# Voyager0587/yolov8-vit

Measured on AMD Instinct MI355X. Metric: images/sec end-to-end (640->224 detect+classify), higher is better.
Workload: dtype bf16; 1 GPU; YOLOv8n(nc=5)+ViT-B/16 end-to-end inference, 640x640, bf16 (BASELINE.json configs[1]); batch_per_gpu=32, global_batch=32, crops_per_image=4, parallelism=dp1, weights=random-init, seed 42

## Files before the change

include/yv_hip.h:

```cpp
#ifndef YV_HIP_H
#define YV_HIP_H

#include <stddef.h>
#include <stdint.h>

#ifdef __cplusplus
extern "C" {
#endif

#define YV_OK 0
#define YV_ERR_ARG (-1)
#define YV_ERR_LIMIT (-2)
#define YV_ERR_WORKSPACE (-3)
#define YV_ERR_LAUNCH (-4)

int yv_version(void);
const char* yv_error_string(int code);
int yv_device_is_gfx950(void);
int yv_set_option(const char* key, int value);
int yv_get_option(const char* key, int* value);

int yv_linear_mxfp8_q(const void* Aq, long long lda, const void* Ascale, long long a_rows_pad, const void* Wq, const void* Wscale,
                      long long w_rows_pad, const float* bias, int M, int N, int K, int flags, const int32_t* m_dev, int m_mul,
                      void* out_q, long long ldq, void* out_scales, long long out_rows_pad, void* stream);
// ... 168 lines not shown
} yv_mx_view;

int yv_quant_mxfp8_map(const void* x, long long ldx, long long pixels, int C, void* q, long long ldq, void* scales,
                       void* stream);

int yv_conv2d_mxfp8(const yv_mx_view* in0, const yv_mx_view* in1, int B, int Hout, int Wout, int ksize, int stride,
                    const void* wq, const void* wscale, long long w_rows_pad, const float* bias, int Cout, void* out_bf16,
                    int out_ld, void* out_q, void* out_scales, int outq_ld, const void* res, int res_ld, int flags,
                    void* stream);
int yv_conv2d_mxfp8_instance(int B, int Hout, int Wout, int ksize, int stride, int Cin, int Cout);

int yv_c2f_fused(const void* x, long long ldx, int B, int H, int W, int c, int n, const void* w_cv1, const float* b_cv1,
                 const void* const* w_m, const float* const* b_m, const void* w_cv2, const float* b_cv2, void* out,
                 long long ldo, void* stream);
int yv_c2f_debug(void* buf);

int yv_conv2d_ws(const yv_view* in0, const yv_view* in1, int B, int Hout, int Wout, int ksize, int stride,
                 const void* weight, const float* bias, int Cout, void* out, int out_ld, const void* res, int res_ld,
                 int flags, void* ws, size_t ws_bytes, void* stream);

int yv_conv2d_stats(const yv_view* in0, int B, int Hout, int Wout, int ksize, int stride, const void* weight,
                    const float* bias, int Cout, void* out, int out_ld, int flags, float* stats_ws, size_t stats_ws_floats,
                    void* ws, size_t ws_bytes, void* stream);
size_t yv_conv_stats_ws_floats(long long T, int Cout);

int yv_conv2d_bnbwd(const yv_view* in0, int B, int Hout, int Wout, int ksize, int stride, const void* weight, const float* bias,
                    int Cout, void* out, int out_ld, const void* res, int res_ld, int flags, const void* z, int ldz,
                    const float* mean, const float* rstd, const float* gamma, const float* beta, int act, float* stats_ws,
                    size_t stats_ws_floats, void* ws, size_t ws_bytes, void* stream);
size_t yv_conv_bnbwd_ws_floats(long long T, int Cout);
// ... 194 lines not shown
```

yolov8-vit_amd/csrc/c2f.hip:

```cpp
#include "yv_common.h"

namespace {

struct C2fArgs {
    const uint16_t* x; long long ldx;
    int B, H, W, tiles_x, tiles_y;
    const uint16_t* w_cv1; const float* b_cv1;
    const uint16_t* w_m[4]; const float* b_m[4];
    const uint16_t* w_cv2; const float* b_cv2;
    uint16_t* out; long long ldo;
    unsigned long long* dbg;
};

__device__ __forceinline__ float c2f_silu(float x) { return x * __builtin_amdgcn_rcpf(1.0f + __expf(-x)); }

typedef __attribute__((ext_vector_type(4))) uint32_t c2f_u32x4;

__device__ __forceinline__ bf16x8 c2f_zero8() { return __builtin_bit_cast(bf16x8, (c2f_u32x4){0u, 0u, 0u, 0u}); }

template <int C, int NB, int TT> struct C2fGeo {
    static constexpr int C2F_T = TT;
    static constexpr int HALO = 2 * NB, R0 = C2F_T + 2 * HALO, PXB = C * 2;
    static constexpr int y_w(int j) { return j == 0 ? C2F_T : R0 - 4 * (j - 1); }
    static constexpr int t_w(int j) { return R0 - 2 - 4 * j; }
    static constexpr int y_off(int j) {
        int o = 0;
        for (int i = 0; i < j; ++i) o += y_w(i) * y_w(i) * PXB + (i >= 1 && i <= NB ? t_w(i - 1) * t_w(i - 1) * PXB : 0);
        return o;
    }
    static constexpr int t_off(int j) { return y_off(j + 1) + y_w(j + 1) * y_w(j + 1) * PXB; }
    static constexpr int BYTES = y_off(NB + 1) + y_w(NB + 1) * y_w(NB + 1) * PXB;
};

template <int C> struct C2fConvW {
    static constexpr int CPG = C / 8, KG = 9 * CPG, KS = (KG + 3) / 4, NFR = C / 16;
    bf16x8 wa[NFR][KS];
    float4 bv[NFR];
};
template <int C>
__device__ __forceinline__ void c2f_load_conv_w(C2fConvW<C>& w, const uint16_t* __restrict__ wgt, const float* __restrict__ bias, int r,
                                                int q) {
    using CW = C2fConvW<C>;
#pragma unroll
    for (int ks = 0; ks < CW::KS; ++ks) {
        const int kg = 4 * ks + q;
#pragma unroll
        for (int f = 0; f < CW::NFR; ++f)
            w.wa[f][ks] = kg < CW::KG ? *(const bf16x8*)(wgt + (size_t)(16 * f + r) * (9 * C) + 8 * kg) : c2f_zero8();
    }
#pragma unroll
    for (int f = 0; f < CW::NFR; ++f) w.bv[f] = *(const float4*)(bias + 16 * f + 4 * q);
}

template <int C, int NTH, bool RES>
__device__ __forceinline__ void c2f_conv3(const C2fConvW<C>& w, const unsigned char* S, int ws, unsigned char* D,
                                          const unsigned char* Rs, int oy, int ox, int H, int W, int lane, int wave) {
    using CW = C2fConvW<C>;
    constexpr int CPG = CW::CPG, KG = CW::KG, KS = CW::KS, NFR = CW::NFR, NW = NTH / 64;
    const int r = lane & 15, q = lane >> 4;
    const int wd = ws - 2, npd = wd * wd, nps = ws * ws, wr = ws + 2;
    int off[KS];
    uint32_t vmask = 0;
#pragma unroll
    for (int ks = 0; ks < KS; ++ks) {
        const int kg = 4 * ks + q;
        const bool valid = kg < KG;
        const int tap = kg / CPG, plane = kg - tap * CPG;
        off[ks] = valid ? ((tap / 3) * ws + (tap % 3) + plane * nps) * 16 : 0;
        vmask |= valid ? 1u << ks : 0u;
    }
    const int ngroups = (npd + 15) >> 4;
    for (int g0 = wave; g0 < ngroups; g0 += 2 * NW) {
        int p_[2], py_[2], px_[2];
        bool live_[2];
        bf16x8 xb[2][KS];
#pragma unroll
        for (int u = 0; u < 2; ++u) {
            const int g = g0 + u * NW;
            live_[u] = g < ngroups;
            const int p = (live_[u] ? g : g0) * 16 + r;
            const int pc = p < npd ? p : npd - 1;
            p_[u] = p; py_[u] = pc / wd; px_[u] = pc - py_[u] * wd;
            const int sbase = (py_[u] * ws + px_[u]) * 16;
#pragma unroll
            for (int ks = 0; ks < KS; ++ks) {
                xb[u][ks] = *(const bf16x8*)(S + sbase + off[ks]);
                if constexpr ((KG & 3) != 0) { if (ks == KS - 1 && !((vmask >> ks) & 1)) xb[u][ks] = c2f_zero8(); }
            }
        }
        f32x4 acc[2][NFR];
#pragma unroll
        for (int u = 0; u < 2; ++u)
#pragma unroll
            for (int f = 0; f < NFR; ++f) acc[u][f] = (f32x4){0.f, 0.f, 0.f, 0.f};
#pragma unroll
        for (int ks = 0; ks < KS; ++ks)
#pragma unroll
            for (int u = 0; u < 2; ++u)
#pragma unroll
                for (int f = 0; f < NFR; ++f)
                    acc[u][f] = __builtin_amdgcn_mfma_f32_16x16x32_bf16(w.wa[f][ks], xb[u][ks], acc[u][f], 0, 0, 0);
#pragma unroll
        for (int u = 0; u < 2; ++u) {
            const int p = p_[u], py = py_[u], px = px_[u];
            const int iy = oy + py, ix = ox + px;
            const bool inimg = iy >= 0 && iy < H && ix >= 0 && ix < W;
#pragma unroll
            for (int f = 0; f < NFR; ++f) {
                const int ch0 = 16 * f + 4 * q;
                float v[4] = {c2f_silu(acc[u][f][0] + w.bv[f].x), c2f_silu(acc[u][f][1] + w.bv[f].y), c2f_silu(acc[u][f][2] + w.bv[f].z),
                              c2f_silu(acc[u][f][3] + w.bv[f].w)};
                if constexpr (RES) {
                    const uint2 rr = *(const uint2*)(Rs + ((ch0 >> 3) * (wr * wr) + (py + 2) * wr + (px + 2)) * 16 + ((ch0 >> 2) & 1) * 8);
                    v[0] += bf16_to_f32((uint16_t)(rr.x & 0xffff)); v[1] += bf16_to_f32((uint16_t)(rr.x >> 16));
                    v[2] += bf16_to_f32((uint16_t)(rr.y & 0xffff)); v[3] += bf16_to_f32((uint16_t)(rr.y >> 16));
                }
                uint2 pk = make_uint2(pack_bf16x2(v[0], v[1]), pack_bf16x2(v[2], v[3]));
                if (!inimg) pk = make_uint2(0u, 0u);
                if (live_[u] && p < npd) *(uint2*)(D + ((ch0 >> 3) * npd + p) * 16 + ((ch0 >> 2) & 1) * 8) = pk;
            }
        }
    }
}

constexpr int C2F_NTH = 256;

template <int C, int NB, int TT>
__global__ __launch_bounds__(C2F_NTH) void c2f_fused_kernel(C2fArgs a) {
    using G = C2fGeo<C, NB, TT>;
    constexpr int T = TT, HALO = G::HALO, R0 = G::R0, CPG = C / 8, C1 = 2 * C, NTH = C2F_NTH, NW = NTH / 64;
    extern __shared__ __attribute__((aligned(16))) unsigned char smem[];
    const int tid = threadIdx.x, lane = tid & 63, wave = __builtin_amdgcn_readfirstlane(tid >> 6);
    const int r = lane & 15, q = lane >> 4;
    int bid = blockIdx.x;
    const int tx = bid % a.tiles_x; bid /= a.tiles_x;
    const int ty = bid % a.tiles_y;
    const int b = bid / a.tiles_y;
    const int H = a.H, W = a.W;
    const int oy = ty * T - HALO, ox = tx * T - HALO;

    C2fConvW<C> wA, wB;
    unsigned long long st_[8] = {0, 0, 0, 0, 0, 0, 0, 0};
    int sti = 0;
    auto stamp = [&]() __attribute__((always_inline)) { if (a.dbg) st_[sti] = __builtin_readcyclecounter(); ++sti; };
    stamp();
    {
        constexpr int NFR = C1 / 16, KS = C1 / 32, N0 = R0 * R0, NG = (N0 + 15) / 16, MAXG = (NG + NW - 1) / NW;
        bf16x8 xb[MAXG][KS];
#pragma unroll
        for (int i = 0; i < MAXG; ++i) {
            const int p = (wave + i * NW) * 16 + r;
            const int py = p / R0, px = p - py * R0;
            const int iy = oy + py, ix = ox + px;
            const bool inimg = p < N0 && iy >= 0 && iy < H && ix >= 0 && ix < W;
            const uint16_t* src = a.x + (((long long)b * H + (inimg ? iy : 0)) * W + (inimg ? ix : 0)) * a.ldx + 8 * q;
#pragma unroll
            for (int ks = 0; ks < KS; ++ks) xb[i][ks] = inimg ? *(const bf16x8*)(src + 32 * ks) : c2f_zero8();
        }
        bf16x8 wa[NFR][KS];
        float4 bv[NFR];
#pragma unroll
        for (int f = 0; f < NFR; ++f) {
#pragma unroll
            for (int ks = 0; ks < KS; ++ks) wa[f][ks] = *(const bf16x8*)(a.w_cv1 + (size_t)(16 * f + r) * C1 + 32 * ks + 8 * q);
            bv[f] = *(const float4*)(a.b_cv1 + 16 * f + 4 * q);
        }
        c2f_load_conv_w<C>(wA, a.w_m[0], a.b_m[0], r, q);
        unsigned char* Y0 = smem + G::y_off(0);
        unsigned char* Y1 = smem + G::y_off(1);
#pragma unroll
        for (int i = 0; i < MAXG; ++i) {
            const int p = (wave + i * NW) * 16 + r;
            const int py = p / R0, px = p - py * R0;
            const int iy = oy + py, ix = ox + px;
            const bool inimg = p < N0 && iy >= 0 && iy < H && ix >= 0 && ix < W;
            f32x4 acc[NFR];
#pragma unroll
            for (int f = 0; f < NFR; ++f) acc[f] = (f32x4){0.f, 0.f, 0.f, 0.f};
#pragma unroll
            for (int ks = 0; ks < KS; ++ks)
#pragma unroll
                for (int f = 0; f < NFR; ++f) acc[f] = __builtin_amdgcn_mfma_f32_16x16x32_bf16(wa[f][ks], xb[i][ks], acc[f], 0, 0, 0);
            const bool centre = py >= HALO && py < HALO + T && px >= HALO && px < HALO + T;
#pragma unroll
            for (int f = 0; f < NFR; ++f) {
                const int ch0 = 16 * f + 4 * q;
                uint2 pk = make_uint2(pack_bf16x2(c2f_silu(acc[f][0] + bv[f].x), c2f_silu(acc[f][1] + bv[f].y)),
                                      pack_bf16x2(c2f_silu(acc[f][2] + bv[f].z), c2f_silu(acc[f][3] + bv[f].w)));
                if (!inimg) pk = make_uint2(0u, 0u);
                if (ch0 < C) {
                    if (centre && p < N0) *(uint2*)(Y0 + ((ch0 >> 3) * (T * T) + (py - HALO) * T + (px - HALO)) * 16 + ((ch0 >> 2) & 1) * 8) = pk;
                } else if (p < N0) {
                    const int c0 = ch0 - C;
                    *(uint2*)(Y1 + ((c0 >> 3) * N0 + p) * 16 + ((c0 >> 2) & 1) * 8) = pk;
                }
            }
        }
    }
    constexpr int NFR2 = C1 / 16, KG2 = (2 + NB) * CPG, KS2 = (KG2 + 3) / 4, KC2 = (2 + NB) * C;
    bf16x8 w2[NFR2][KS2];
    float4 bv2[NFR2];
    auto load_w2 = [&]() __attribute__((always_inline)) {
#pragma unroll
        for (int ks = 0; ks < KS2; ++ks) {
            const int kg = 4 * ks + q;
#pragma unroll
            for (int f = 0; f < NFR2; ++f)
                w2[f][ks] = kg < KG2 ? *(const bf16x8*)(a.w_cv2 + (size_t)(16 * f + r) * KC2 + 8 * kg) : c2f_zero8();
        }
#pragma unroll
        for (int f = 0; f < NFR2; ++f) bv2[f] = *(const float4*)(a.b_cv2 + 16 * f + 4 * q);
    };
    c2f_load_conv_w<C>(wB, a.w_m[1], a.b_m[1], r, q);
    stamp();
    __syncthreads();
    stamp();
    c2f_conv3<C, NTH, false>(wA, smem + G::y_off(1), G::y_w(1), smem + G::t_off(0), nullptr, oy + 1, ox + 1, H, W, lane, wave);
    if constexpr (NB == 2) c2f_load_conv_w<C>(wA, a.w_m[2], a.b_m[2], r, q); else load_w2();
    stamp();
    __syncthreads();
    c2f_conv3<C, NTH, true>(wB, smem + G::t_off(0), G::t_w(0), smem + G::y_off(2), smem + G::y_off(1), oy + 2, ox + 2, H, W, lane, wave);
    if constexpr (NB == 2) {
        c2f_load_conv_w<C>(wB, a.w_m[3], a.b_m[3], r, q);
        __syncthreads();
        c2f_conv3<C, NTH, false>(wA, smem + G::y_off(2), G::y_w(2), smem + G::t_off(1), nullptr, oy + 3, ox + 3, H, W, lane, wave);
        load_w2();
        __syncthreads();
        c2f_conv3<C, NTH, true>(wB, smem + G::t_off(1), G::t_w(1), smem + G::y_off(3), smem + G::y_off(2), oy + 4, ox + 4, H, W, lane, wave);
    }
    stamp();
    __syncthreads();
    stamp();
    {
        int cbase[KS2], cw[KS2];
        uint32_t vmask = 0;
#pragma unroll
        for (int ks = 0; ks < KS2; ++ks) {
            const int kg = 4 * ks + q;
            const bool valid = kg < KG2;
            vmask |= valid ? 1u << ks : 0u;
            const int arr = kg / CPG, plane = kg - arr * CPG;
            int w_ = T, co = 0, base = G::y_off(0);
            if (arr == 1) { w_ = G::y_w(1); co = HALO; base = G::y_off(1); }
            else if (arr == 2) { w_ = G::y_w(2); co = HALO - 2; base = G::y_off(2); }
            else if (arr == 3) { w_ = G::y_w(NB + 1); co = HALO - 4; base = G::y_off(NB + 1); }
            cw[ks] = w_;
            cbase[ks] = valid ? base + (plane * w_ * w_ + co * w_ + co) * 16 : 0;
        }
        constexpr int NG2 = T * T / 16;
        for (int g0 = wave; g0 < NG2; g0 += 2 * NW) {
            bf16x8 xb[2][KS2];
            bool live_[2];
            int p_[2];
#pragma unroll
            for (int u = 0; u < 2; ++u) {
                live_[u] = g0 + u * NW < NG2;
                const int p = (live_[u] ? g0 + u * NW : g0) * 16 + r;
                p_[u] = p;
                const int py = p / T, px = p - py * T;
#pragma unroll
                for (int ks = 0; ks < KS2; ++ks) {
                    xb[u][ks] = *(const bf16x8*)(smem + cbase[ks] + (py * cw[ks] + px) * 16);
                    if constexpr ((KG2 & 3) != 0) { if (ks == KS2 - 1 && !((vmask >> ks) & 1)) xb[u][ks] = c2f_zero8(); }
                }
            }
            f32x4 acc[2][NFR2];
#pragma unroll
            for (int u = 0; u < 2; ++u)
#pragma unroll
                for (int f = 0; f < NFR2; ++f) acc[u][f] = (f32x4){0.f, 0.f, 0.f, 0.f};
#pragma unroll
            for (int ks = 0; ks < KS2; ++ks)
#pragma unroll
                for (int u = 0; u < 2; ++u)
#pragma unroll
                    for (int f = 0; f < NFR2; ++f)
                        acc[u][f] = __builtin_amdgcn_mfma_f32_16x16x32_bf16(w2[f][ks], xb[u][ks], acc[u][f], 0, 0, 0);
#pragma unroll
            for (int u = 0; u < 2; ++u) {
                const int p = p_[u];
                const int py = p / T, px = p - py * T;
                const int iy = ty * T + py, ix = tx * T + px;
                if (live_[u] && iy < H && ix < W) {
                    uint16_t* dst = a.out + (((long long)b * H + iy) * W + ix) * a.ldo + 4 * q;
#pragma unroll
                    for (int f = 0; f < NFR2; ++f)
                        *(uint2*)(dst + 16 * f) = make_uint2(pack_bf16x2(c2f_silu(acc[u][f][0] + bv2[f].x), c2f_silu(acc[u][f][1] + bv2[f].y)),
                                                             pack_bf16x2(c2f_silu(acc[u][f][2] + bv2[f].z), c2f_silu(acc[u][f][3] + bv2[f].w)));
                }
            }
        }
    }
    stamp();
    if (a.dbg && lane == 0 && wave == 0 && blockIdx.x < 64) {
#pragma unroll
        for (int i = 0; i < 8; ++i) a.dbg[blockIdx.x * 8 + i] = st_[i];
    }
}

template <int C, int NB, int TT>
int launch_c2f(C2fArgs& a, hipStream_t st) {
    constexpr int lds = C2fGeo<C, NB, TT>::BYTES;
    static_assert(lds <= 160 * 1024, "LDS");
    if (!yv_grant_lds((const void*)c2f_fused_kernel<C, NB, TT>, lds)) return YV_ERR_LAUNCH;
    a.tiles_x = (a.W + TT - 1) / TT; a.tiles_y = (a.H + TT - 1) / TT;
    const long long grid = (long long)a.tiles_x * a.tiles_y * a.B;
    if (grid > 0x7fffffffLL) return YV_ERR_LIMIT;
    hipLaunchKernelGGL((c2f_fused_kernel<C, NB, TT>), dim3((unsigned)grid), dim3(C2F_NTH), lds, st, a);
    return yv_launch_status();
}
unsigned long long* g_c2f_dbg = nullptr;

}

extern "C" int yv_c2f_debug(void* buf) { g_c2f_dbg = (unsigned long long*)buf; return YV_OK; }

extern "C" int yv_c2f_fused(const void* x, long long ldx, int B, int H, int W, int c, int n, const void* w_cv1, const float* b_cv1,
                            const void* const* w_m, const float* const* b_m, const void* w_cv2, const float* b_cv2, void* out,
                            long long ldo, void* stream) {
    if (!x || !w_cv1 || !b_cv1 || !w_m || !b_m || !w_cv2 || !b_cv2 || !out || B <= 0 || H <= 0 || W <= 0) return YV_ERR_ARG;
    if ((c != 16 && c != 32) || (n != 1 && n != 2)) return YV_ERR_ARG;
    if (ldx < 2 * c || ldo < 2 * c || (ldx & 7) || (ldo & 3) || (((uintptr_t)x | (uintptr_t)w_cv1 | (uintptr_t)w_cv2) & 15) ||
        ((uintptr_t)out & 7) || (((uintptr_t)b_cv1 | (uintptr_t)b_cv2) & 15))
        return YV_ERR_ARG;
    C2fArgs a = {};
    a.x = (const uint16_t*)x; a.ldx = ldx; a.B = B; a.H = H; a.W = W;
    a.w_cv1 = (const uint16_t*)w_cv1; a.b_cv1 = b_cv1; a.w_cv2 = (const uint16_t*)w_cv2; a.b_cv2 = b_cv2;
    for (int j = 0; j < 2 * n; ++j) {
        if (!w_m[j] || !b_m[j] || ((uintptr_t)w_m[j] & 15) || ((uintptr_t)b_m[j] & 15)) return YV_ERR_ARG;
        a.w_m[j] = (const uint16_t*)w_m[j]; a.b_m[j] = b_m[j];
    }
    a.out = (uint16_t*)out; a.ldo = ldo; a.dbg = g_c2f_dbg;
    hipStream_t st = (hipStream_t)stream;
    if (c == 16) return n == 1 ? launch_c2f<16, 1, 16>(a, st) : launch_c2f<16, 2, 16>(a, st);
    return n == 1 ? launch_c2f<32, 1, 16>(a, st) : launch_c2f<32, 2, 16>(a, st);
}
```

yolov8-vit_amd/csrc/yolo_misc.hip:

```cpp
#include "yv_common.h"

namespace {

template <int COUT>
__global__ __launch_bounds__(256) void stem_kernel(const uint8_t* __restrict__ img, int H, int W,
                                                   const float* __restrict__ wgt, const float* __restrict__ bias,
                                                   uint16_t* __restrict__ out, int out_ld, long long npix) {
    const int Ho = H >> 1, Wo = W >> 1;
    const long long p = (long long)blockIdx.x * 256 + threadIdx.x;
    if (p >= npix) return;
    const int b = (int)(p / ((long long)Ho * Wo));
    const int rem = (int)(p - (long long)b * Ho * Wo);
    const int oy = rem / Wo, ox = rem - oy * Wo;
    float x[27];
    const uint8_t* src = img + (size_t)b * H * W * 3;
#pragma unroll
    for (int ky = 0; ky < 3; ++ky)
#pragma unroll
        for (int kx = 0; kx < 3; ++kx) {
            const int iy = oy * 2 + ky - 1, ix = ox * 2 + kx - 1;
            const bool ok = iy >= 0 && iy < H && ix >= 0 && ix < W;
            const uint8_t* px = src + ((size_t)(ok ? iy : 0) * W + (ok ? ix : 0)) * 3;
#pragma unroll
            for (int c = 0; c < 3; ++c) x[(ky * 3 + kx) * 3 + c] = ok ? (float)px[c] * (1.0f / 255.0f) : 0.f;
// ... 3 lines not shown
    for (int cg = 0; cg < COUT; cg += 8) {
        float acc[8];
#pragma unroll
        for (int q = 0; q < 8; ++q) acc[q] = bias[cg + q];
#pragma unroll
        for (int k = 0; k < 27; ++k)
#pragma unroll
            for (int q = 0; q < 8; ++q) acc[q] = fmaf(x[k], wgt[k * COUT + cg + q], acc[q]);
#pragma unroll
        for (int q = 0; q < 8; ++q) acc[q] = acc[q] * __builtin_amdgcn_rcpf(1.0f + __expf(-acc[q]));
        *(uint4*)(o + cg) = make_uint4(pack_bf16x2(acc[0], acc[1]), pack_bf16x2(acc[2], acc[3]),
                                       pack_bf16x2(acc[4], acc[5]), pack_bf16x2(acc[6], acc[7]));
    }
}

template <int COUT>
__global__ __launch_bounds__(256) void stem_mfma_kernel(const uint8_t* __restrict__ img, int H, int W,
                                                        const float* __restrict__ wgt, const float* __restrict__ bias,
                                                        uint16_t* __restrict__ out, int out_ld, int chunks) {
    constexpr int NFR = COUT / 16;
    __shared__ __attribute__((aligned(16))) unsigned char stage[4 * 3 * 512];
    const int lane = threadIdx.x & 63, wave = threadIdx.x >> 6;
    const int fr = lane & 15, fq = lane >> 4;
    const int Ho = H >> 1, Wo = W >> 1, cpr = Wo >> 6;
    bf16x8 wh[NFR], wl[NFR];
    float4 bv[NFR];
#pragma unroll
    for (int i = 0; i < NFR; ++i) {
        uint32_t ph[4], pl[4];
#pragma unroll
        for (int q2 = 0; q2 < 4; ++q2) {
// ... 25 lines not shown
    unsigned char* win = stage + wave * (3 * 512);
#pragma unroll
    for (int ky = 0; ky < 3; ++ky) {
        const int iy = 2 * oy + ky - 1;
        const int xo = xa + lane * 8;
        const uint32_t o = (iy >= 0 && xo >= 0 && xo + 8 <= rowb) ? (uint32_t)(iy * rowb + xo) : OOB;
        const u32x2 d = __builtin_amdgcn_raw_buffer_load_b64(rs, o, 0, 0);
        *(u32x2*)(win + ky * 512 + lane * 8) = d;
    }
    int loff[8];
#pragma unroll
    for (int q = 0; q < 8; ++q) {
        const int ky = fq < 3 ? fq : (q < 3 ? q : 0), t = fq < 3 ? q : 8;
        loff[q] = ky * 512 + t - xa;
    }
#pragma unroll
    for (int g = 0; g < 4; ++g) {
        const int ox = c64 * 64 + g * 16 + fr;
        const int xb = 6 * ox - 3;
        uint32_t v[8];
#pragma unroll
        for (int q = 0; q < 8; ++q) {
            const uint32_t byte = (fq < 3 || q < 3) ? (uint32_t)win[loff[q] + xb] : 0u;
            v[q] = __float_as_uint((float)byte);
        }
        uint32_t pk[4];
#pragma unroll
        for (int q2 = 0; q2 < 4; ++q2)
            pk[q2] = __builtin_amdgcn_perm(v[2 * q2 + 1], v[2 * q2], 0x07060302u);
        const u32x4 pa = {pk[0], pk[1], pk[2], pk[3]};
        const bf16x8 fa = __builtin_bit_cast(bf16x8, pa);
        uint16_t* o = out + ((size_t)row * Wo + ox) * out_ld + fq * 4;
#pragma unroll
        for (int i = 0; i < NFR; ++i) {
            f32x4 acc = {0.f, 0.f, 0.f, 0.f};
            acc = __builtin_amdgcn_mfma_f32_16x16x32_bf16(wh[i], fa, acc, 0, 0, 0);
            acc = __builtin_amdgcn_mfma_f32_16x16x32_bf16(wl[i], fa, acc, 0, 0, 0);
            float r[4] = {acc[0] + bv[i].x, acc[1] + bv[i].y, acc[2] + bv[i].z, acc[3] + bv[i].w};
#pragma unroll
// ... 39 lines not shown
                if (yy < 0 || yy >= H) continue;
                for (int dx = -2; dx <= 2; ++dx) {
                    const int xx = x + dx;
                    if (xx < 0 || xx >= W) continue;
                    max8(m, in[yy * W + xx]);
                }
            }
            const uint4 v = pack8(m);
            outp[i] = v;
            *(uint4*)(base + (size_t)i * ld + (stage + 1) * c) = v;
        }
        __syncthreads();
    }
}

}

extern "C" int yv_stem_conv(const uint8_t* images, int B, int H, int W, const float* weight, const float* bias,
                            int Cout, void* out, int out_ld, void* stream) {
    if (!images || !weight || !bias || !out || B <= 0 || H <= 0 || W <= 0) return YV_ERR_ARG;
    if ((H & 1) || (W & 1) || (out_ld & 7) || out_ld < Cout) return YV_ERR_ARG;
    if (Cout != 16 && Cout != 32 && Cout != 48) return YV_ERR_LIMIT;
    const long long npix = (long long)B * (H / 2) * (W / 2);
    const dim3 grid((unsigned)((npix + 255) / 256)), block(256);
    hipStream_t st = (hipStream_t)stream;
    uint16_t* o = (uint16_t*)out;
    if ((W % 128) == 0 && npix < 0x7fffffffLL && (long long)H * W * 3 < 0x7fffffffLL && ((uintptr_t)images & 7) == 0) {
        const int chunks = (int)(npix / 64);
        const int blocks = (chunks + 3) / 4;
        const dim3 g4((unsigned)(blocks < 2048 ? blocks : 2048));
        if (Cout == 16) hipLaunchKernelGGL(stem_mfma_kernel<16>, g4, block, 0, st, images, H, W, weight, bias, o, out_ld, chunks);
        else if (Cout == 32) hipLaunchKernelGGL(stem_mfma_kernel<32>, g4, block, 0, st, images, H, W, weight, bias, o, out_ld, chunks);
        else hipLaunchKernelGGL(stem_mfma_kernel<48>, g4, block, 0, st, images, H, W, weight, bias, o, out_ld, chunks);
        return yv_launch_status();
    }
    if (Cout == 16) hipLaunchKernelGGL(stem_kernel<16>, grid, block, 0, st, images, H, W, weight, bias, o, out_ld, npix);
    else if (Cout == 32) hipLaunchKernelGGL(stem_kernel<32>, grid, block, 0, st, images, H, W, weight, bias, o, out_ld, npix);
    else hipLaunchKernelGGL(stem_kernel<48>, grid, block, 0, st, images, H, W, weight, bias, o, out_ld, npix);
    return yv_launch_status();
}

extern "C" int yv_sppf_pool(void* buf, int B, int H, int W, int ld, int c, void* stream) {
    if (!buf || B <= 0 || H <= 0 || W <= 0 || c <= 0) return YV_ERR_ARG;
    if ((c & 7) || (ld & 7) || ld < 4 * c) return YV_ERR_ARG;
    if (H * W > SPPF_MAX_HW) return YV_ERR_LIMIT;
    hipLaunchKernelGGL(sppf_kernel, dim3(B * (c / 8)), dim3(512), 0, (hipStream_t)stream, (uint16_t*)buf, H, W, ld, c);
    return yv_launch_status();
}
```

yolov8-vit_amd/yvhip/__init__.py:

```python
from __future__ import annotations

import collections
import ctypes as C
import os

_HWQ_PRESET = os.environ.get("GPU_MAX_HW_QUEUES")
os.environ.setdefault("GPU_MAX_HW_QUEUES", "8")
import re
from typing import List, Optional, Tuple

import torch

HW_QUEUES = int(_HWQ_PRESET) if _HWQ_PRESET else (4 if torch.cuda.is_initialized() else 8)

_HERE = os.path.dirname(os.path.abspath(__file__))
LIB_PATH = os.path.join(_HERE, "libyvhip.so")
HEADER_PATH = os.path.normpath(os.path.join(_HERE, "..", "..", "include", "yv_hip.h"))


class YvError(RuntimeError):
    pass


from .extent import n_anchors, net_hw
# ... 69 lines not shown
                                 _vp, _vp, _vp, _vp, _vp, _vp, _vp]),
    "yv_compact_crops": (_i, [_vp, _vp, _vp, _i, _i, _i, _vp, _vp, _vp]),
    "yv_compact_crops_split": (_i, [_vp, _vp, _vp, _i, _i, _i, _i, _vp, _vp, _vp]),
    "yv_crop_resize_norm": (_i, [_vp, _i, _i, _i, _sz, _vp, _vp, _i, _i, _i, _i, _vp, _vp]),
    "yv_letterbox": (_i, [_vp, _i, _i, _i, _vp, _i, _vp, _vp]),
    "yv_letterbox_hw": (_i, [_vp, _i, _i, _i, _vp, _i, _i, _vp, _vp]),
    "yv_augment_patchify": (_i, [_vp, _i, _i, _i, _vp, _vp, _vp, _vp]),
    "yv_train_crops": (_i, [_vp, _sz, _vp, _i, _vp, _i, _i, _i, _vp, _vp, _i, _vp, _vp]),
    "yv_mosaic_augment": (_i, [_vp, _i, _i, _i, _vp, _vp, _vp, _vp, _vp]),
    "yv_mosaic_augment_ex": (_i, [_vp, _i, _i, _i, _i, _vp, _vp, _vp, _vp, _vp, _vp]),
    "yv_detect_decode": (_i, [_vp, _vp, _vp, _vp, _vp, _vp, _i, _i, _i, _i, _vp, _vp, _vp]),
    "yv_detect_tail": (_i, [_vp, _vp, _vp, _i, _i, _vp, _vp, _vp, _vp, _i, _i, _i, _vp, _vp, _vp]),
    "yv_detect_decode_hw": (_i, [_vp, _vp, _vp, _vp, _vp, _vp, _i, _i, _i, _i, _i, _vp, _vp, _vp]),
    "yv_detect_tail_hw": (_i, [_vp, _vp, _vp, _i, _i, _vp, _vp, _vp, _vp, _i, _i, _i, _i, _vp, _vp, _vp]),
    "yv_c2f_debug": (_i, [_vp]),
    "yv_crop_debug": (_i, [_i]),
    "yv_c2f_fused": (_i, [_vp, C.c_longlong, _i, _i, _i, _i, _i, _vp, _vp, _vp, _vp, _vp, _vp, _vp, C.c_longlong, _vp]),
    "yv_optim_step": (_i, [_i, _vp, _vp, _vp, _vp, _sz, _f, _f, _f, _f, _f, _f, _i, _vp, _vp]),
    "yv_optim_step_rec": (_i, [_i, _vp, _vp, _vp, _vp, _sz, _f, _f, _f, _f, _f, _vp, _i, _vp, _vp]),
    "yv_grad_clip_ws_bytes": (_sz, [_sz]),
    "yv_grad_clip_record": (_i, [_vp, _sz, _f, _f, _vp, _sz, _vp, _vp, _vp]),
    "yv_ema_update": (_i, [_vp, _vp, _sz, _f, _vp]),
    "yv_axpby": (_i, [_vp, _vp, _sz, _f, _f, _vp]),
    "yv_detect_loss_ws_bytes": (_sz, [_i, _i, _i]),
    "yv_detect_loss": (_i, [_vp, _vp, _vp, _vp, _i, _i, _i, _i, _vp, _vp, _vp, _i, _f, _f, _f, _vp, _vp, _sz, _vp]),
    "yv_blob_nhwc8": (_i, [_vp, C.c_longlong, _vp, _vp]),
    "yv_bn_ws_floats": (_sz, [C.c_longlong, _i]),
    "yv_bn_stats": (_i, [_vp, C.c_longlong, C.c_longlong, _i, _f, _f, _vp, _vp, _vp, _vp, _vp, _sz, _vp]),
    "yv_bn_stats_finish": (_i, [_vp, C.c_longlong, _i, _f, _f, _vp, _vp, _vp, _vp, _vp]),
    "yv_conv_stats_ws_floats": (_sz, [C.c_longlong, _i]),
# ... 405 lines not shown
    scores = torch.empty((B, A, nc), dtype=torch.float32, device=dev)
    check(lib.yv_detect_tail(_p(feats[0]), _p(feats[1]), _p(feats[2]), ld, c3, arr(w2), arr(b2), arr(w3), arr(b3), B, size, nc,
                             _p(boxes), _p(scores), _st()), "yv_detect_tail")
    return boxes, scores


def c2f_fused(x: torch.Tensor, c: int, n: int, w_cv1, b_cv1, w_m, b_m, w_cv2, b_cv2, out: torch.Tensor):
    _chk_dev(x, out, w_cv1, b_cv1, w_cv2, b_cv2, *w_m, *b_m)
    B, H, W = x.shape[0], x.shape[1], x.shape[2]
    arr = lambda ts: (C.c_void_p * len(ts))(*[t.data_ptr() for t in ts])
    check(lib.yv_c2f_fused(_p(x), x.stride(2), B, H, W, c, n, _p(w_cv1), _p(b_cv1), arr(w_m), arr(b_m), _p(w_cv2), _p(b_cv2),
                           _p(out), out.stride(2), _st()), "yv_c2f_fused")
    return out


def loss_fwd_bwd(logits: torch.Tensor, labels: torch.Tensor, w_lsce: float = 1.0 / 6.0, w_focal: float = 5.0 / 6.0):
    _chk_dev(logits, labels)
    B, nc = logits.shape
    loss = torch.empty((1,), dtype=torch.float32, device=logits.device)
    grad = torch.empty_like(logits)
    check(lib.yv_loss_fwd_bwd(_p(logits), _p(labels), B, nc, float(w_lsce), float(w_focal), _p(loss), _p(grad), _st()),
          "yv_loss_fwd_bwd")
    return loss, grad


def sgd_step(p: torch.Tensor, g: torch.Tensor, m: torch.Tensor, lr: float, momentum: float = 0.9,
             weight_decay: float = 1e-3, first: bool = False, grad_scale: float = 1.0,
             mirror: Optional[torch.Tensor] = None, scale_rec: Optional[torch.Tensor] = None):
    _chk_dev(p, g, m, mirror)
    if scale_rec is not None:
# ... 950 lines not shown
```

Measured before the change: 4749 images/s.

## Add two-workgroup C2f tiling, word-aligned stem loads, separable SPPF pooling

New measurement: 4765 images/s (median of 6 runs). About the same (+0.4%).

```diff
diff --git a/include/yv_hip.h b/include/yv_hip.h
--- a/include/yv_hip.h
+++ b/include/yv_hip.h
@@ -206,6 +206,10 @@
                  const void* const* w_m, const float* const* b_m, const void* w_cv2, const float* b_cv2, void* out,
                  long long ldo, void* stream);
 int yv_c2f_debug(void* buf);
+#define YV_FORM_C2F 1
+#define YV_FORM_STEM 2
+#define YV_FORM_SPPF 4
+int yv_detector_parent_forms(int mask);
 
 int yv_conv2d_ws(const yv_view* in0, const yv_view* in1, int B, int Hout, int Wout, int ksize, int stride,
                  const void* weight, const float* bias, int Cout, void* out, int out_ld, const void* res, int res_ld,
diff --git a/yolov8-vit_amd/csrc/c2f.hip b/yolov8-vit_amd/csrc/c2f.hip
--- a/yolov8-vit_amd/csrc/c2f.hip
+++ b/yolov8-vit_amd/csrc/c2f.hip
@@ -18,18 +18,21 @@
 
 __device__ __forceinline__ bf16x8 c2f_zero8() { return __builtin_bit_cast(bf16x8, (c2f_u32x4){0u, 0u, 0u, 0u}); }
 
-template <int C, int NB, int TT> struct C2fGeo {
-    static constexpr int C2F_T = TT;
-    static constexpr int HALO = 2 * NB, R0 = C2F_T + 2 * HALO, PXB = C * 2;
-    static constexpr int y_w(int j) { return j == 0 ? C2F_T : R0 - 4 * (j - 1); }
-    static constexpr int t_w(int j) { return R0 - 2 - 4 * j; }
+template <int C, int NB, int TX, int TY, bool OVL> struct C2fGeo {
+    static constexpr int HALO = 2 * NB, RX = TX + 2 * HALO, RY = TY + 2 * HALO, PXB = C * 2;
+    static constexpr int y_wx(int j) { return j == 0 ? TX : RX - 4 * (j - 1); }
+    static constexpr int y_wy(int j) { return j == 0 ? TY : RY - 4 * (j - 1); }
+    static constexpr int t_wx(int j) { return RX - 2 - 4 * j; }
+    static constexpr int t_wy(int j) { return RY - 2 - 4 * j; }
+    static constexpr int y_bytes(int j) { return y_wx(j) * y_wy(j) * PXB; }
+    static constexpr int t_bytes(int j) { return OVL && j >= 1 ? 0 : t_wx(j) * t_wy(j) * PXB; }
     static constexpr int y_off(int j) {
         int o = 0;
-        for (int i = 0; i < j; ++i) o += y_w(i) * y_w(i) * PXB + (i >= 1 && i <= NB ? t_w(i - 1) * t_w(i - 1) * PXB : 0);
+        for (int i = 0; i < j; ++i) o += y_bytes(i) + (i >= 1 && i <= NB ? t_bytes(i - 1) : 0);
         return o;
     }
-    static constexpr int t_off(int j) { return y_off(j + 1) + y_w(j + 1) * y_w(j + 1) * PXB; }
-    static constexpr int BYTES = y_off(NB + 1) + y_w(NB + 1) * y_w(NB + 1) * PXB;
+    static constexpr int t_off(int j) { return OVL && j >= 1 ? y_off(1) + y_bytes(1) : y_off(j + 1) + y_bytes(j + 1); }
+    static constexpr int BYTES = y_off(NB + 1) + y_bytes(NB + 1);
 };
 
 template <int C> struct C2fConvW {
@@ -52,13 +55,13 @@
     for (int f = 0; f < CW::NFR; ++f) w.bv[f] = *(const float4*)(bias + 16 * f + 4 * q);
 }
 
-template <int C, int NTH, bool RES>
-__device__ __forceinline__ void c2f_conv3(const C2fConvW<C>& w, const unsigned char* S, int ws, unsigned char* D,
+template <int C, int NTH, bool RES, int U>
+__device__ __forceinline__ void c2f_conv3(const C2fConvW<C>& w, const unsigned char* S, int ws, int hs, unsigned char* D,
                                           const unsigned char* Rs, int oy, int ox, int H, int W, int lane, int wave) {
     using CW = C2fConvW<C>;
     constexpr int CPG = CW::CPG, KG = CW::KG, KS = CW::KS, NFR = CW::NFR, NW = NTH / 64;
     const int r = lane & 15, q = lane >> 4;
-    const int wd = ws - 2, npd = wd * wd, nps = ws * ws, wr = ws + 2;
+    const int wd = ws - 2, npd = wd * (hs - 2), nps = ws * hs, wr = ws + 2, npr = wr * (hs + 2);
     int off[KS];
     uint32_t vmask = 0;
 #pragma unroll
@@ -70,12 +73,12 @@
         vmask |= valid ? 1u << ks : 0u;
     }
     const int ngroups = (npd + 15) >> 4;
-    for (int g0 = wave; g0 < ngroups; g0 += 2 * NW) {
-        int p_[2], py_[2], px_[2];
-        bool live_[2];
-        bf16x8 xb[2][KS];
-#pragma unroll
-        for (int u = 0; u < 2; ++u) {
+    for (int g0 = wave; g0 < ngroups; g0 += U * NW) {
+        int p_[U], py_[U], px_[U];
+        bool live_[U];
+        bf16x8 xb[U][KS];
+#pragma unroll
+        for (int u = 0; u < U; ++u) {
             const int g = g0 + u * NW;
             live_[u] = g < ngroups;
             const int p = (live_[u] ? g : g0) * 16 + r;
@@ -88,20 +91,20 @@
                 if constexpr ((KG & 3) != 0) { if (ks == KS - 1 && !((vmask >> ks) & 1)) xb[u][ks] = c2f_zero8(); }
             }
         }
-        f32x4 acc[2][NFR];
-#pragma unroll
-        for (int u = 0; u < 2; ++u)
+        f32x4 acc[U][NFR];
+#pragma unroll
+        for (int u = 0; u < U; ++u)
 #pragma unroll
             for (int f = 0; f < NFR; ++f) acc[u][f] = (f32x4){0.f, 0.f, 0.f, 0.f};
 #pragma unroll
         for (int ks = 0; ks < KS; ++ks)
 #pragma unroll
-            for (int u = 0; u < 2; ++u)
+            for (int u = 0; u < U; ++u)
 #pragma unroll
                 for (int f = 0; f < NFR; ++f)
                     acc[u][f] = __builtin_amdgcn_mfma_f32_16x16x32_bf16(w.wa[f][ks], xb[u][ks], acc[u][f], 0, 0, 0);
 #pragma unroll
-        for (int u = 0; u < 2; ++u) {
+        for (int u = 0; u < U; ++u) {
             const int p = p_[u], py = py_[u], px = px_[u];
             const int iy = oy + py, ix = ox + px;
             const bool inimg = iy >= 0 && iy < H && ix >= 0 && ix < W;
@@ -111,7 +114,7 @@
                 float v[4] = {c2f_silu(acc[u][f][0] + w.bv[f].x), c2f_silu(acc[u][f][1] + w.bv[f].y), c2f_silu(acc[u][f][2] + w.bv[f].z),
                               c2f_silu(acc[u][f][3] + w.bv[f].w)};
                 if constexpr (RES) {
-                    const uint2 rr = *(const uint2*)(Rs + ((ch0 >> 3) * (wr * wr) + (py + 2) * wr + (px + 2)) * 16 + ((ch0 >> 2) & 1) * 8);
+                    const uint2 rr = *(const uint2*)(Rs + ((ch0 >> 3) * npr + (py + 2) * wr + (px + 2)) * 16 + ((ch0 >> 2) & 1) * 8);
                     v[0] += bf16_to_f32((uint16_t)(rr.x & 0xffff)); v[1] += bf16_to_f32((uint16_t)(rr.x >> 16));
                     v[2] += bf16_to_f32((uint16_t)(rr.y & 0xffff)); v[3] += bf16_to_f32((uint16_t)(rr.y >> 16));
                 }
@@ -125,10 +128,10 @@
 
 constexpr int C2F_NTH = 256;
 
-template <int C, int NB, int TT>
-__global__ __launch_bounds__(C2F_NTH) void c2f_fused_kernel(C2fArgs a) {
-    using G = C2fGeo<C, NB, TT>;
-    constexpr int T = TT, HALO = G::HALO, R0 = G::R0, CPG = C / 8, C1 = 2 * C, NTH = C2F_NTH, NW = NTH / 64;
+template <int C, int NB, int TX, int TY, int U, bool TWO_WG>
+__device__ __forceinline__ void c2f_block(C2fArgs a) {
+    using G = C2fGeo<C, NB, TX, TY, TWO_WG>;
+    constexpr int HALO = G::HALO, RX = G::RX, RY = G::RY, CPG = C / 8, C1 = 2 * C, NTH = C2F_NTH, NW = NTH / 64;
     extern __shared__ __attribute__((aligned(16))) unsigned char smem[];
     const int tid = threadIdx.x, lane = tid & 63, wave = __builtin_amdgcn_readfirstlane(tid >> 6);
     const int r = lane & 15, q = lane >> 4;
@@ -137,7 +140,7 @@
     const int ty = bid % a.tiles_y;
     const int b = bid / a.tiles_y;
     const int H = a.H, W = a.W;
-    const int oy = ty * T - HALO, ox = tx * T - HALO;
+    const int oy = ty * TY - HALO, ox = tx * TX - HALO;
 
     C2fConvW<C> wA, wB;
     unsigned long long st_[8] = {0, 0, 0, 0, 0, 0, 0, 0};
@@ -145,12 +148,12 @@
     auto stamp = [&]() __attribute__((always_inline)) { if (a.dbg) st_[sti] = __builtin_readcyclecounter(); ++sti; };
     stamp();
     {
-        constexpr int NFR = C1 / 16, KS = C1 / 32, N0 = R0 * R0, NG = (N0 + 15) / 16, MAXG = (NG + NW - 1) / NW;
+        constexpr int NFR = C1 / 16, KS = C1 / 32, N0 = RX * RY, NG = (N0 + 15) / 16, MAXG = (NG + NW - 1) / NW;
         bf16x8 xb[MAXG][KS];
 #pragma unroll
         for (int i = 0; i < MAXG; ++i) {
             const int p = (wave + i * NW) * 16 + r;
-            const int py = p / R0, px = p - py * R0;
+            const int py = p / RX, px = p - py * RX;
             const int iy = oy + py, ix = ox + px;
             const bool inimg = p < N0 && iy >= 0 && iy < H && ix >= 0 && ix < W;
             const uint16_t* src = a.x + (((long long)b * H + (inimg ? iy : 0)) * W + (inimg ? ix : 0)) * a.ldx + 8 * q;
@@ -171,7 +174,7 @@
 #pragma unroll
         for (int i = 0; i < MAXG; ++i) {
             const int p = (wave + i * NW) * 16 + r;
-            const int py = p / R0, px = p - py * R0;
+            const int py = p / RX, px = p - py * RX;
             const int iy = oy + py, ix = ox + px;
             const bool inimg = p < N0 && iy >= 0 && iy < H && ix >= 0 && ix < W;
             f32x4 acc[NFR];
@@ -181,7 +184,7 @@
             for (int ks = 0; ks < KS; ++ks)
 #pragma unroll
                 for (int f = 0; f < NFR; ++f) acc[f] = __builtin_amdgcn_mfma_f32_16x16x32_bf16(wa[f][ks], xb[i][ks], acc[f], 0, 0, 0);
-            const bool centre = py >= HALO && py < HALO + T && px >= HALO && px < HALO + T;
+            const bool centre = py >= HALO && py < HALO + TY && px >= HALO && px < HALO + TX;
 #pragma unroll
             for (int f = 0; f < NFR; ++f) {
                 const int ch0 = 16 * f + 4 * q;
@@ -189,7 +192,7 @@
                                       pack_bf16x2(c2f_silu(acc[f][2] + bv[f].z), c2f_silu(acc[f][3] + bv[f].w)));
                 if (!inimg) pk = make_uint2(0u, 0u);
                 if (ch0 < C) {
-                    if (centre && p < N0) *(uint2*)(Y0 + ((ch0 >> 3) * (T * T) + (py - HALO) * T + (px - HALO)) * 16 + ((ch0 >> 2) & 1) * 8) = pk;
+                    if (centre && p < N0) *(uint2*)(Y0 + ((ch0 >> 3) * (TX * TY) + (py - HALO) * TX + (px - HALO)) * 16 + ((ch0 >> 2) & 1) * 8) = pk;
                 } else if (p < N0) {
                     const int c0 = ch0 - C;
                     *(uint2*)(Y1 + ((c0 >> 3) * N0 + p) * 16 + ((c0 >> 2) & 1) * 8) = pk;
@@ -211,22 +214,42 @@
 #pragma unroll
         for (int f = 0; f < NFR2; ++f) bv2[f] = *(const float4*)(a.b_cv2 + 16 * f + 4 * q);
     };
-    c2f_load_conv_w<C>(wB, a.w_m[1], a.b_m[1], r, q);
-    stamp();
-    __syncthreads();
-    stamp();
-    c2f_conv3<C, NTH, false>(wA, smem + G::y_off(1), G::y_w(1), smem + G::t_off(0), nullptr, oy + 1, ox + 1, H, W, lane, wave);
-    if constexpr (NB == 2) c2f_load_conv_w<C>(wA, a.w_m[2], a.b_m[2], r, q); else load_w2();
-    stamp();
-    __syncthreads();
-    c2f_conv3<C, NTH, true>(wB, smem + G::t_off(0), G::t_w(0), smem + G::y_off(2), smem + G::y_off(1), oy + 2, ox + 2, H, W, lane, wave);
-    if constexpr (NB == 2) {
-        c2f_load_conv_w<C>(wB, a.w_m[3], a.b_m[3], r, q);
+    if constexpr (!TWO_WG) {
+        c2f_load_conv_w<C>(wB, a.w_m[1], a.b_m[1], r, q);
+        stamp();
         __syncthreads();
-        c2f_conv3<C, NTH, false>(wA, smem + G::y_off(2), G::y_w(2), smem + G::t_off(1), nullptr, oy + 3, ox + 3, H, W, lane, wave);
+        stamp();
+        c2f_conv3<C, NTH, false, U>(wA, smem + G::y_off(1), G::y_wx(1), G::y_wy(1), smem + G::t_off(0), nullptr, oy + 1, ox + 1, H, W, lane, wave);
+        if constexpr (NB == 2) c2f_load_conv_w<C>(wA, a.w_m[2], a.b_m[2], r, q); else load_w2();
+        stamp();
+        __syncthreads();
+        c2f_conv3<C, NTH, true, U>(wB, smem + G::t_off(0), G::t_wx(0), G::t_wy(0), smem + G::y_off(2), smem + G::y_off(1), oy + 2, ox + 2, H, W, lane, wave);
+        if constexpr (NB == 2) {
+            c2f_load_conv_w<C>(wB, a.w_m[3], a.b_m[3], r, q);
+            __syncthreads();
+            c2f_conv3<C, NTH, false, U>(wA, smem + G::y_off(2), G::y_wx(2), G::y_wy(2), smem + G::t_off(1), nullptr, oy + 3, ox + 3, H, W, lane, wave);
+            load_w2();
+            __syncthreads();
+            c2f_conv3<C, NTH, true, U>(wB, smem + G::t_off(1), G::t_wx(1), G::t_wy(1), smem + G::y_off(3), smem + G::y_off(2), oy + 4, ox + 4, H, W, lane, wave);
+        }
+    } else {
+        stamp();
+        __syncthreads();
+        stamp();
+        c2f_conv3<C, NTH, false, U>(wA, smem + G::y_off(1), G::y_wx(1), G::y_wy(1), smem + G::t_off(0), nullptr, oy + 1, ox + 1, H, W, lane, wave);
+        c2f_load_conv_w<C>(wA, a.w_m[1], a.b_m[1], r, q);
+        stamp();
+        __syncthreads();
+        c2f_conv3<C, NTH, true, U>(wA, smem + G::t_off(0), G::t_wx(0), G::t_wy(0), smem + G::y_off(2), smem + G::y_off(1), oy + 2, ox + 2, H, W, lane, wave);
+        if constexpr (NB == 2) {
+            c2f_load_conv_w<C>(wA, a.w_m[2], a.b_m[2], r, q);
+            __syncthreads();
+            c2f_conv3<C, NTH, false, U>(wA, smem + G::y_off(2), G::y_wx(2), G::y_wy(2), smem + G::t_off(1), nullptr, oy + 3, ox + 3, H, W, lane, wave);
+            c2f_load_conv_w<C>(wA, a.w_m[3], a.b_m[3], r, q);
+            __syncthreads();
+            c2f_conv3<C, NTH, true, U>(wA, smem + G::t_off(1), G::t_wx(1), G::t_wy(1), smem + G::y_off(3), smem + G::y_off(2), oy + 4, ox + 4, H, W, lane, wave);
+        }
         load_w2();
-        __syncthreads();
-        c2f_conv3<C, NTH, true>(wB, smem + G::t_off(1), G::t_w(1), smem + G::y_off(3), smem + G::y_off(2), oy + 4, ox + 4, H, W, lane, wave);
     }
     stamp();
     __syncthreads();
@@ -240,14 +263,14 @@
             const bool valid = kg < KG2;
             vmask |= valid ? 1u << ks : 0u;
             const int arr = kg / CPG, plane = kg - arr * CPG;
-            int w_ = T, co = 0, base = G::y_off(0);
-            if (arr == 1) { w_ = G::y_w(1); co = HALO; base = G::y_off(1); }
-            else if (arr == 2) { w_ = G::y_w(2); co = HALO - 2; base = G::y_off(2); }
-            else if (arr == 3) { w_ = G::y_w(NB + 1); co = HALO - 4; base = G::y_off(NB + 1); }
+            int w_ = TX, co = 0, base = G::y_off(0);
+            if (arr == 1) { w_ = G::y_wx(1); co = HALO; base = G::y_off(1); }
+            else if (arr == 2) { w_ = G::y_wx(2); co = HALO - 2; base = G::y_off(2); }
+            else if (arr == 3) { w_ = G::y_wx(NB + 1); co = HALO - 4; base = G::y_off(NB + 1); }
             cw[ks] = w_;
-            cbase[ks] = valid ? base + (plane * w_ * w_ + co * w_ + co) * 16 : 0;
-        }
-        constexpr int NG2 = T * T / 16;
+            cbase[ks] = valid ? base + (plane * w_ * (w_ + (TY - TX)) + co * w_ + co) * 16 : 0;
+        }
+        constexpr int NG2 = TX * TY / 16;
         for (int g0 = wave; g0 < NG2; g0 += 2 * NW) {
             bf16x8 xb[2][KS2];
             bool live_[2];
@@ -257,7 +280,7 @@
                 live_[u] = g0 + u * NW < NG2;
                 const int p = (live_[u] ? g0 + u * NW : g0) * 16 + r;
                 p_[u] = p;
-                const int py = p / T, px = p - py * T;
+                const int py = p / TX, px = p - py * TX;
 #pragma unroll
                 for (int ks = 0; ks < KS2; ++ks) {
                     xb[u][ks] = *(const bf16x8*)(smem + cbase[ks] + (py * cw[ks] + px) * 16);
@@ -279,8 +302,8 @@
 #pragma unroll
             for (int u = 0; u < 2; ++u) {
                 const int p = p_[u];
-                const int py = p / T, px = p - py * T;
-                const int iy = ty * T + py, ix = tx * T + px;
+                const int py = p / TX, px = p - py * TX;
+                const int iy = ty * TY + py, ix = tx * TX + px;
                 if (live_[u] && iy < H && ix < W) {
                     uint16_t* dst = a.out + (((long long)b * H + iy) * W + ix) * a.ldo + 4 * q;
 #pragma unroll
@@ -299,19 +322,39 @@
 }
 
 template <int C, int NB, int TT>
-int launch_c2f(C2fArgs& a, hipStream_t st) {
-    constexpr int lds = C2fGeo<C, NB, TT>::BYTES;
-    static_assert(lds <= 160 * 1024, "LDS");
-    if (!yv_grant_lds((const void*)c2f_fused_kernel<C, NB, TT>, lds)) return YV_ERR_LAUNCH;
-    a.tiles_x = (a.W + TT - 1) / TT; a.tiles_y = (a.H + TT - 1) / TT;
+__global__ __launch_bounds__(C2F_NTH) void c2f_fused_kernel(C2fArgs a) { c2f_block<C, NB, TT, TT, 2, false>(a); }
+
+constexpr int C2F_TX2 = 16, C2F_TY2 = 8, C2F_U2 = 1;
+template <int C, int NB>
+__global__ __launch_bounds__(C2F_NTH, 2) void c2f_fused2_kernel(C2fArgs a) { c2f_block<C, NB, C2F_TX2, C2F_TY2, C2F_U2, true>(a); }
+
+template <int LDS, typename K>
+int launch_c2f_tiles(K kernel, int tx, int ty, C2fArgs& a, hipStream_t st) {
+    if (!yv_grant_lds((const void*)kernel, LDS)) return YV_ERR_LAUNCH;
+    a.tiles_x = (a.W + tx - 1) / tx; a.tiles_y = (a.H + ty - 1) / ty;
     const long long grid = (long long)a.tiles_x * a.tiles_y * a.B;
     if (grid > 0x7fffffffLL) return YV_ERR_LIMIT;
-    hipLaunchKernelGGL((c2f_fused_kernel<C, NB, TT>), dim3((unsigned)grid), dim3(C2F_NTH), lds, st, a);
+    hipLaunchKernelGGL(kernel, dim3((unsigned)grid), dim3(C2F_NTH), LDS, st, a);
     return yv_launch_status();
 }
+template <int C, int NB, int TT>
+int launch_c2f(C2fArgs& a, hipStream_t st) {
+    constexpr int lds = C2fGeo<C, NB, TT, TT, false>::BYTES;
+    static_assert(lds <= 160 * 1024, "LDS");
+    return launch_c2f_tiles<lds>(c2f_fused_kernel<C, NB, TT>, TT, TT, a, st);
+}
+template <int C, int NB>
+int launch_c2f2(C2fArgs& a, hipStream_t st) {
+    using G = C2fGeo<C, NB, C2F_TX2, C2F_TY2, true>;
+    static_assert(G::BYTES <= 80 * 1024, "LDS: two workgroups per CU");
+    static_assert(NB < 2 || G::t_wx(1) * G::t_wy(1) <= G::t_wx(0) * G::t_wy(0), "t1 lies over t0");
+    return launch_c2f_tiles<G::BYTES>(c2f_fused2_kernel<C, NB>, C2F_TX2, C2F_TY2, a, st);
+}
 unsigned long long* g_c2f_dbg = nullptr;
 
 }
+
+extern int yv_detector_parent_forms_mask;
 
 extern "C" int yv_c2f_debug(void* buf) { g_c2f_dbg = (unsigned long long*)buf; return YV_OK; }
 
@@ -333,5 +376,6 @@
     a.out = (uint16_t*)out; a.ldo = ldo; a.dbg = g_c2f_dbg;
     hipStream_t st = (hipStream_t)stream;
     if (c == 16) return n == 1 ? launch_c2f<16, 1, 16>(a, st) : launch_c2f<16, 2, 16>(a, st);
-    return n == 1 ? launch_c2f<32, 1, 16>(a, st) : launch_c2f<32, 2, 16>(a, st);
-}
+    if (n == 1) return launch_c2f<32, 1, 16>(a, st);
+    return (yv_detector_parent_forms_mask & YV_FORM_C2F) ? launch_c2f<32, 2, 16>(a, st) : launch_c2f2<32, 2>(a, st);
+}
diff --git a/yolov8-vit_amd/csrc/yolo_misc.hip b/yolov8-vit_amd/csrc/yolo_misc.hip
--- a/yolov8-vit_amd/csrc/yolo_misc.hip
+++ b/yolov8-vit_amd/csrc/yolo_misc.hip
@@ -41,7 +41,7 @@
     }
 }
 
-template <int COUT>
+template <int COUT, bool BYTES>
 __global__ __launch_bounds__(256) void stem_mfma_kernel(const uint8_t* __restrict__ img, int H, int W,
                                                         const float* __restrict__ wgt, const float* __restrict__ bias,
                                                         uint16_t* __restrict__ out, int out_ld, int chunks) {
@@ -97,15 +97,30 @@
         const int ky = fq < 3 ? fq : (q < 3 ? q : 0), t = fq < 3 ? q : 8;
         loff[q] = ky * 512 + t - xa;
     }
+    const int first = 6 * fr + (x0 - xa) + (fq < 3 ? 0 : 8);
+    const int wbase = (fq < 3 ? fq * 512 : 0) + (first & ~3), wstep = fq < 3 ? 4 : 512, shift = first & 3;
 #pragma unroll
     for (int g = 0; g < 4; ++g) {
         const int ox = c64 * 64 + g * 16 + fr;
         const int xb = 6 * ox - 3;
         uint32_t v[8];
-#pragma unroll
-        for (int q = 0; q < 8; ++q) {
-            const uint32_t byte = (fq < 3 || q < 3) ? (uint32_t)win[loff[q] + xb] : 0u;
-            v[q] = __float_as_uint((float)byte);
+        if constexpr (BYTES) {
+#pragma unroll
+            for (int q = 0; q < 8; ++q) {
+                const uint32_t byte = (fq < 3 || q < 3) ? (uint32_t)win[loff[q] + xb] : 0u;
+                v[q] = __float_as_uint((float)byte);
+            }
+        } else {
+            uint32_t w[3];
+#pragma unroll
+            for (int k = 0; k < 3; ++k) w[k] = *(const uint32_t*)(win + wbase + 96 * g + k * wstep);
+            uint32_t lo = __builtin_amdgcn_alignbyte(w[1], w[0], shift), hi = __builtin_amdgcn_alignbyte(w[2], w[1], shift);
+            if (fq == 3) {
+                lo = ((w[0] >> (8 * shift)) & 0xffu) | (((w[1] >> (8 * shift)) & 0xffu) << 8) | (((w[2] >> (8 * shift)) & 0xffu) << 16);
+                hi = 0u;
+            }
+#pragma unroll
+            for (int q = 0; q < 8; ++q) v[q] = __float_as_uint((float)(((q < 4 ? lo : hi) >> (8 * (q & 3))) & 0xffu));
         }
         uint32_t pk[4];
 #pragma unroll
@@ -175,6 +190,48 @@
     }
 }
 
+__global__ __launch_bounds__(512) void sppf_sep_kernel(uint16_t* __restrict__ buf, int H, int W, int ld, int c) {
+    __shared__ uint4 plane[2][SPPF_MAX_HW];
+    const int cgs = c >> 3;
+    const int b = blockIdx.x / cgs, cg = blockIdx.x - b * cgs;
+    const int hw = H * W;
+    uint16_t* base = buf + (size_t)b * hw * ld + cg * 8;
+    for (int i = threadIdx.x; i < hw; i += blockDim.x) plane[0][i] = *(const uint4*)(base + (size_t)i * ld);
+    __syncthreads();
+    for (int stage = 0; stage < 3; ++stage) {
+        for (int i = threadIdx.x; i < hw; i += blockDim.x) {
+            const int y = i / W, x = i - y * W;
+            float m[8];
+#pragma unroll
+            for (int q = 0; q < 8; ++q) m[q] = -INFINITY;
+#pragma unroll
+            for (int dx = -2; dx <= 2; ++dx) max8(m, plane[0][y * W + min(max(x + dx, 0), W - 1)]);
+            plane[1][i] = pack8(m);
+        }
+        __syncthreads();
+        for (int i = threadIdx.x; i < hw; i += blockDim.x) {
+            const int y = i / W, x = i - y * W;
+            float m[8];
+#pragma unroll
+            for (int q = 0; q < 8; ++q) m[q] = -INFINITY;
+#pragma unroll
+            for (int dy = -2; dy <= 2; ++dy) max8(m, plane[1][min(max(y + dy, 0), H - 1) * W + x]);
+            const uint4 v = pack8(m);
+            plane[0][i] = v;
+            *(uint4*)(base + (size_t)i * ld + (stage + 1) * c) = v;
+        }
+        __syncthreads();
+    }
+}
+
+}
+
+int yv_detector_parent_forms_mask = 0;
+
+extern "C" int yv_detector_parent_forms(int mask) {
+    if (mask & ~(YV_FORM_C2F | YV_FORM_STEM | YV_FORM_SPPF)) return YV_ERR_ARG;
+    yv_detector_parent_forms_mask = mask;
+    return YV_OK;
 }
 
 extern "C" int yv_stem_conv(const uint8_t* images, int B, int H, int W, const float* weight, const float* bias,
@@ -190,9 +247,11 @@
         const int chunks = (int)(npix / 64);
         const int blocks = (chunks + 3) / 4;
         const dim3 g4((unsigned)(blocks < 2048 ? blocks : 2048));
-        if (Cout == 16) hipLaunchKernelGGL(stem_mfma_kernel<16>, g4, block, 0, st, images, H, W, weight, bias, o, out_ld, chunks);
-        else if (Cout == 32) hipLaunchKernelGGL(stem_mfma_kernel<32>, g4, block, 0, st, images, H, W, weight, bias, o, out_ld, chunks);
-        else hipLaunchKernelGGL(stem_mfma_kernel<48>, g4, block, 0, st, images, H, W, weight, bias, o, out_ld, chunks);
+        const bool bytes = yv_detector_parent_forms_mask & YV_FORM_STEM;
+        auto launch = [&](auto kernel) { hipLaunchKernelGGL(kernel, g4, block, 0, st, images, H, W, weight, bias, o, out_ld, chunks); };
+        if (Cout == 16) launch(bytes ? stem_mfma_kernel<16, true> : stem_mfma_kernel<16, false>);
+        else if (Cout == 32) launch(bytes ? stem_mfma_kernel<32, true> : stem_mfma_kernel<32, false>);
+        else launch(bytes ? stem_mfma_kernel<48, true> : stem_mfma_kernel<48, false>);
         return yv_launch_status();
     }
     if (Cout == 16) hipLaunchKernelGGL(stem_kernel<16>, grid, block, 0, st, images, H, W, weight, bias, o, out_ld, npix);
@@ -205,6 +264,7 @@
     if (!buf || B <= 0 || H <= 0 || W <= 0 || c <= 0) return YV_ERR_ARG;
     if ((c & 7) || (ld & 7) || ld < 4 * c) return YV_ERR_ARG;
     if (H * W > SPPF_MAX_HW) return YV_ERR_LIMIT;
-    hipLaunchKernelGGL(sppf_kernel, dim3(B * (c / 8)), dim3(512), 0, (hipStream_t)stream, (uint16_t*)buf, H, W, ld, c);
+    const auto kernel = (yv_detector_parent_forms_mask & YV_FORM_SPPF) ? sppf_kernel : sppf_sep_kernel;
+    hipLaunchKernelGGL(kernel, dim3(B * (c / 8)), dim3(512), 0, (hipStream_t)stream, (uint16_t*)buf, H, W, ld, c);
     return yv_launch_status();
 }
diff --git a/yolov8-vit_amd/yvhip/__init__.py b/yolov8-vit_amd/yvhip/__init__.py
--- a/yolov8-vit_amd/yvhip/__init__.py
+++ b/yolov8-vit_amd/yvhip/__init__.py
@@ -107,6 +107,7 @@
     "yv_detect_decode_hw": (_i, [_vp, _vp, _vp, _vp, _vp, _vp, _i, _i, _i, _i, _i, _vp, _vp, _vp]),
     "yv_detect_tail_hw": (_i, [_vp, _vp, _vp, _i, _i, _vp, _vp, _vp, _vp, _i, _i, _i, _i, _vp, _vp, _vp]),
     "yv_c2f_debug": (_i, [_vp]),
+    "yv_detector_parent_forms": (_i, [_i]),
     "yv_crop_debug": (_i, [_i]),
     "yv_c2f_fused": (_i, [_vp, C.c_longlong, _i, _i, _i, _i, _i, _vp, _vp, _vp, _vp, _vp, _vp, _vp, C.c_longlong, _vp]),
     "yv_optim_step": (_i, [_i, _vp, _vp, _vp, _vp, _sz, _f, _f, _f, _f, _f, _f, _i, _vp, _vp]),
@@ -542,6 +543,13 @@
     return out
 
 
+FORM_C2F, FORM_STEM, FORM_SPPF = 1, 2, 4
+
+
+def detector_parent_forms(mask: int = 0):
+    check(lib.yv_detector_parent_forms(mask), "yv_detector_parent_forms")
+
+
 def loss_fwd_bwd(logits: torch.Tensor, labels: torch.Tensor, w_lsce: float = 1.0 / 6.0, w_focal: float = 5.0 / 6.0):
     _chk_dev(logits, labels)
     B, nc = logits.shape
```
